# houchenfeng/4DGaussians-fast-train

Hardware: AMD Instinct MI355X
Metric: train-step ms + rasterizer fwd+bwd MGaussians/s @100k pts, 1352×1014 (higher is better)
Workload: dtype f32; 1 GPU; metric: P=100000 Gaussians, 1352x1014, SH deg 3, 1 view/GPU/step, fwd+bwd; global_batch=1, parallelism=views x1 (independent views + RCCL loss all-reduce)

## Files before the change

4dgaussians-fast-train_amd/csrc/capi.hip:

```cpp
#include <stdio.h>
#include <string.h>

#include <algorithm>
#include <string>
#include <vector>

#include "../../include/gs4d.h"
#include "gs4d_internal.h"

namespace gs4d {

static thread_local std::string g_last_error;
static thread_local bool g_profiling = false;
static thread_local int g_stage_repeats = 1;
static thread_local std::vector<std::pair<const char *, hipEvent_t>> g_marks;
static thread_local std::vector<int> g_mark_div;
static thread_local std::vector<std::pair<const char *, float>> g_timings;

static int fail(int code, const std::string &msg) {
    g_last_error = msg;
    return code;
}
int train_fail(int code, const std::string &msg) { return fail(code, msg); }

#define GS4D_HIP(expr)                                                                                                  \
    do {                                                                                                               \
        hipError_t e_ = (expr);                                                                                        \
        if (e_ != hipSuccess)                                                                                          \
            return fail(GS4D_ERR_HIP, std::string(#expr) + ": " + hipGetErrorString(e_));                               \
    } while (0)

#define GS4D_STAGE(name, expr)                                                                                          \
    do {                                                                                                               \
        GS4D_HIP(expr);                                                                                                \
        if (debug) {                                                                                                   \
            hipError_t e_ = hipStreamSynchronize(stream);                                                              \
            if (e_ != hipSuccess)                                                                                      \
                return fail(GS4D_ERR_HIP, std::string("[HIP ERROR] in stage ") + name + ": " + hipGetErrorString(e_)); \
        }                                                                                                              \
        mark(name, stream);                                                                                            \
    } while (0)

#define GS4D_REPEATED_STAGE(name, expr)                                                                                 \
    do {                                                                                                               \
        const int reps_ = g_profiling ? g_stage_repeats : 1;                                                           \
        if (reps_ > 1) mark(name "_pre", stream);                                                                      \
        for (int r_ = 0; r_ < reps_; r_++) GS4D_HIP(expr);                                                             \
        if (debug) {                                                                                                   \
            hipError_t e_ = hipStreamSynchronize(stream);                                                              \
            if (e_ != hipSuccess)                                                                                      \
                return fail(GS4D_ERR_HIP, std::string("[HIP ERROR] in stage ") + name + ": " + hipGetErrorString(e_)); \
        }                                                                                                              \
        mark(name, stream, reps_);                                                                                     \
    } while (0)

static void mark(const char *name, hipStream_t s, int div = 1) {
    if (!g_profiling) return;
    hipEvent_t ev;
    if (hipEventCreate(&ev) != hipSuccess) return;
    (void)hipEventRecord(ev, s);
    g_marks.emplace_back(name, ev);
    g_mark_div.push_back(div);
}
static void begin_marks(hipStream_t s) {
    for (auto &m : g_marks) (void)hipEventDestroy(m.second);
    g_marks.clear();
    g_mark_div.clear();
    mark("begin", s);
}
static void end_marks() {
    if (!g_profiling || g_marks.empty()) return;
    (void)hipEventSynchronize(g_marks.back().second);
    g_timings.clear();
    for (size_t i = 1; i < g_marks.size(); i++) {
        float ms = 0.f;
        (void)hipEventElapsedTime(&ms, g_marks[i - 1].second, g_marks[i].second);
        g_timings.emplace_back(g_marks[i].first, ms / (float)g_mark_div[i]);
    }
    for (auto &m : g_marks) (void)hipEventDestroy(m.second);
    g_marks.clear();
    g_mark_div.clear();
}

static char *carve(char *&p, size_t bytes) {
    char *r = p;
    p += align_up(bytes, 256);
    return r;
}

size_t GeomState::required(int P, int T) { return (size_t)carve(nullptr, P, T).zero + 4 * geom_zero_words(P) + 512; }
GeomState GeomState::carve(char *base, int P, int T) {
    char *p = (char *)align_up((size_t)base, 256);
    const size_t n = (size_t)P;
    GeomState g;
    g.depths = (float *)gs4d::carve(p, 4 * n);
    g.radii = (int *)gs4d::carve(p, 4 * n);
    g.xy = (float2 *)gs4d::carve(p, 8 * n);
    g.conic_opacity = (float4 *)gs4d::carve(p, 16 * n);
    g.splat = (float4 *)gs4d::carve(p, 48 * n);
    g.cov3D = (float *)gs4d::carve(p, 24 * n);
    g.clamped = (uint8_t *)gs4d::carve(p, n);
    g.tiles_touched = (uint32_t *)gs4d::carve(p, 4 * n);
    g.n_inst = (uint32_t *)gs4d::carve(p, 4 * n);
    g.vis_gid = (uint32_t *)gs4d::carve(p, 4 * n);
    g.cand_off = (uint32_t *)gs4d::carve(p, 4 * n + 4);
    g.first_vis = (uint32_t *)gs4d::carve(p, 4 * max_emit_chunks(P, T));
    g.emit_chain = (uint32_t *)gs4d::carve(p, 4 * (max_emit_chunks(P, T) + 64));
    g.zero = (uint32_t *)gs4d::carve(p, 4 * geom_zero_words(P));
    return g;
}

size_t ImageState::required(int W, int H) { return (size_t)carve(nullptr, W, H).order + 4 * (size_t)((W + 15) / 16) * ((H + 15) / 16) + 512; }
ImageState ImageState::carve(char *base, int W, int H) {
    char *p = (char *)align_up((size_t)base, 256);
    const size_t N = (size_t)W * H;
    const size_t T = (size_t)((W + kBlockX - 1) / kBlockX) * ((H + kBlockY - 1) / kBlockY);
    ImageState s;
    s.final_T = (float *)gs4d::carve(p, 4 * N);
    s.n_contrib = (uint32_t *)gs4d::carve(p, 4 * N);
    s.ranges = (uint2 *)gs4d::carve(p, 8 * T);
    s.order = (uint32_t *)gs4d::carve(p, 4 * T);
    return s;
}

static uint32_t higher_msb(uint32_t n) {
    uint32_t msb = sizeof(n) * 4;
    uint32_t step = msb;
    while (step > 1) {
        step /= 2;
        if (n >> msb) msb += step; else msb -= step;
    }
    if (n >> msb) msb++;
    return msb;
}

size_t BinningState::required(int L, int T) {
    BinningState b = carve(nullptr, L, T);
    return (size_t)b.scratch + 4 * binning_zero_words(L, T) + 512;
}
BinningState BinningState::carve(char *base, int L, int T) {
    char *p = (char *)align_up((size_t)base, 256);
    BinningState b;
    b.key_bits = (int)higher_msb((uint32_t)T);
    for (int i = 0; i < 2; i++) {
        b.keys[i] = (uint32_t *)gs4d::carve(p, 4 * (size_t)L);
        b.vals[i] = (uint32_t *)gs4d::carve(p, 4 * (size_t)L);
    }
    b.gid_by_e = (uint32_t *)gs4d::carve(p, 4 * (size_t)L);
    const int final_buf = ((b.key_bits + 7) / 8) & 1;
    b.upos = b.vals[final_buf];
    b.sorted_keys = b.keys[final_buf];
    b.tmp_hi = b.keys[final_buf ^ 1];
    b.tmp_lo = b.vals[final_buf ^ 1];
    b.count_items = gs4d::count_items(L, T);
    b.tile_hist = b.count_items ? (uint32_t *)gs4d::carve(p, 4 * tile_hist_words(L, T)) : nullptr;
    b.scratch = (uint32_t *)gs4d::carve(p, 4 * binning_zero_words(L, T));
    return b;
}

static Args make_args(int P, int D, int M, int W, int H, const float *bg, float scale_modifier, const float *view,
                      const float *proj, const float *campos, float tan_fovx, float tan_fovy, int prefiltered) {
    Args a;
    memset(&a, 0, sizeof(a));
    a.P = P; a.D = D; a.M = M; a.W = W; a.H = H;
    a.gx = (W + kBlockX - 1) / kBlockX;
    a.gy = (H + kBlockY - 1) / kBlockY;
    a.scale_modifier = scale_modifier;
    a.tan_fovx = tan_fovx;
    a.tan_fovy = tan_fovy;
    a.focal_y = H / (2.0f * tan_fovy);
    a.focal_x = W / (2.0f * tan_fovx);
    a.viewmatrix = view;
    a.projmatrix = proj;
    a.campos = campos;
    a.bg = bg;
    a.prefiltered = prefiltered;
    return a;
}

}

using namespace gs4d;

extern "C" {

const char *gs4d_last_error(void) { return g_last_error.c_str(); }
const char *gs4d_version(void) { return "gs4d 0.1.0 gfx950"; }
void gs4d_set_profiling(int enabled) {
    g_profiling = enabled != 0;
    g_stage_repeats = enabled >= 2 ? enabled : 1;
// ... 31 lines not shown
                         uint8_t *present, void *stream_, int view_transposed) {
    hipStream_t stream = (hipStream_t)stream_;
    if (P < 0 || (P > 0 && (!means3D || !viewmatrix || !present))) return fail(GS4D_ERR_ARG, "mark_visible: bad args");
    if (P == 0) return GS4D_OK;
    GS4D_HIP(launch_mark_visible(P, means3D, viewmatrix, view_transposed ? 1 : 0, present, stream));
    return GS4D_OK;
}
int gs4d_mark_visible(int P, const float *means3D, const float *viewmatrix, const float *projmatrix,
                      uint8_t *present, void *stream) {
    return gs4d_mark_visible_ex(P, means3D, viewmatrix, projmatrix, present, stream, 0);
}

int gs4d_debug_effective_opacity(int P, const char *geometry_buffer, float *out, void *stream_) {
    if (P < 0 || (P > 0 && (!geometry_buffer || !out))) return fail(GS4D_ERR_ARG, "debug_effective_opacity: bad args");
    if (P == 0) return GS4D_OK;
    GeomState g = GeomState::carve(const_cast<char *>(geometry_buffer), P, 1);
    GS4D_HIP(launch_effective_opacity(P, g, out, (hipStream_t)stream_));
    return GS4D_OK;
}

int gs4d_debug_tile_lists(int P, int width, int height, int num_rendered, const char *geometry_buffer,
                          const char *binning_buffer, const char *image_buffer, uint32_t *ranges, uint32_t *order,
                          uint32_t *n_emitted, uint32_t *gid, uint32_t *reach, uint32_t *slot, float *depth,
                          void *stream_) {
    hipStream_t stream = (hipStream_t)stream_;
    const int R = num_rendered;
    if (P <= 0 || width <= 0 || height <= 0 || R < 0 || !geometry_buffer || !image_buffer || !ranges || !order ||
        !n_emitted || (R > 0 && (!binning_buffer || !gid || !reach || !slot || !depth)))
        return fail(GS4D_ERR_ARG, "debug_tile_lists: bad args");
    const int T = ((width + kBlockX - 1) / kBlockX) * ((height + kBlockY - 1) / kBlockY);
    GeomState g = GeomState::carve(const_cast<char *>(geometry_buffer), P, T);
    ImageState img = ImageState::carve(const_cast<char *>(image_buffer), width, height);
    GS4D_HIP(hipMemcpyAsync(ranges, img.ranges, sizeof(uint2) * (size_t)T, hipMemcpyDeviceToDevice, stream));
    GS4D_HIP(hipMemcpyAsync(order, img.order, 4 * (size_t)T, hipMemcpyDeviceToDevice, stream));
    if (R == 0) {
        GS4D_HIP(hipMemsetAsync(n_emitted, 0, 4, stream));
        return GS4D_OK;
    }
    BinningState b = BinningState::carve(const_cast<char *>(binning_buffer), R, T);
    GS4D_HIP(hipMemcpyAsync(n_emitted, b.scratch, 4, hipMemcpyDeviceToDevice, stream));
    GS4D_HIP(launch_tile_lists(P, R, g, b, gid, reach, slot, depth, stream));
    return GS4D_OK;
}

int gs4d_forward_aa(gs4d_alloc_fn geometry_alloc, void *geometry_ctx, gs4d_alloc_fn binning_alloc, void *binning_ctx,
                    gs4d_alloc_fn image_alloc, void *image_ctx, int P, int D, int M, const float *background,
                    int width, int height, const float *means3D, const float *shs, const float *colors_precomp,
                    const float *opacities, const float *scales, float scale_modifier, const float *rotations,
                    const float *cov3D_precomp, const float *viewmatrix, const float *projmatrix,
                    const float *cam_pos, float tan_fovx, float tan_fovy, int prefiltered, float *out_color,
                    float *out_depth, int *radii, int debug, void *stream_, int *num_rendered, int view_transposed,
                    int antialiasing) {
    hipStream_t stream = (hipStream_t)stream_;
    *num_rendered = 0;
    if (P < 0 || width <= 0 || height <= 0) return fail(GS4D_ERR_ARG, "forward: P must be >= 0 and the image non-empty");
    if (P == 0) return GS4D_OK;
    if (P >= (1 << 30)) return fail(GS4D_ERR_ARG, "forward: at most 2^30 Gaussians");
    if (!means3D || !opacities || !viewmatrix || !projmatrix || !background || !out_color || !out_depth)
        return fail(GS4D_ERR_ARG, "forward: missing required input");
    if (!colors_precomp && (!shs || !cam_pos))
        return fail(GS4D_ERR_ARG, "forward: provide either SHs (+campos) or precomputed colors");
    if (!colors_precomp && (D < 0 || D > 3 || (D + 1) * (D + 1) > M))
        return fail(GS4D_ERR_ARG, "forward: SH degree must be in [0,3] with (D+1)^2 <= M coefficients");
    if (!cov3D_precomp && (!scales || !rotations))
        return fail(GS4D_ERR_ARG, "forward: provide either scales+rotations or precomputed 3D covariances");
    if (((size_t)rotations & 15) != 0 && rotations) return fail(GS4D_ERR_ARG, "forward: rotations must be 16-byte aligned");

    Args a = make_args(P, D, M, width, height, background, scale_modifier, viewmatrix, projmatrix, cam_pos, tan_fovx,
                       tan_fovy, prefiltered);
    a.view_transposed = view_transposed ? 1 : 0;
    begin_marks(stream);

    if ((int64_t)a.gx * a.gy >= (int64_t)1 << 30) return fail(GS4D_ERR_ARG, "forward: at most 2^30 - 1 tiles");
    const int T = a.gx * a.gy;
    a.exact_div = T >= (1 << 20);
    char *gbuf = geometry_alloc(geometry_ctx, GeomState::required(P, T) + 16);
    if (!gbuf) return fail(GS4D_ERR_ALLOC, "forward: geometry buffer allocation failed");
    GeomState g = GeomState::carve(gbuf, P, T);
    char *ibuf = image_alloc(image_ctx, ImageState::required(width, height));
    if (!ibuf) return fail(GS4D_ERR_ALLOC, "forward: image buffer allocation failed");
    ImageState img = ImageState::carve(ibuf, width, height);
    int *radii_ptr = radii ? radii : g.radii;

    GS4D_HIP(hipMemsetAsync(g.zero, 0, 4 * geom_zero_words(P), stream));
    GS4D_STAGE("preprocess", launch_preprocess(a, means3D, scales, rotations, opacities, shs, cov3D_precomp,
                                               colors_precomp, radii_ptr, g, (int *)(g.zero + kZeroFlag),
                                               antialiasing != 0, stream));

    struct Readback {
        uint32_t *pinned = nullptr;
        hipEvent_t copied = nullptr;
    };
    static thread_local Readback readback[kMaxDevices];
    int dev = 0;
    GS4D_HIP(hipGetDevice(&dev));
    if (dev < 0 || dev >= kMaxDevices) return fail(GS4D_ERR_ARG, "forward: device index out of range");
    Readback &rb = readback[dev];
    if (!rb.pinned) GS4D_HIP(hipHostMalloc((void **)&rb.pinned, 128, hipHostMallocDefault));
    if (!rb.copied) GS4D_HIP(hipEventCreateWithFlags(&rb.copied, hipEventDisableTiming));
    uint32_t *pinned = rb.pinned;
    hipEvent_t copied = rb.copied;
    GS4D_HIP(hipMemcpyAsync(pinned, g.zero, 4 * (kZeroL + 16), hipMemcpyDeviceToHost, stream));
    GS4D_HIP(hipEventRecord(copied, stream));
    GS4D_STAGE("visible_scan", launch_visible_scan(a, g, stream));
    GS4D_HIP(hipEventSynchronize(copied));
    if (prefiltered && pinned[kZeroFlag] != 0)
        return fail(GS4D_ERR_PREFILTERED, "Point is filtered although prefiltered is set. This shouldn't happen!");
    uint64_t L64 = 0;
    for (int i = 0; i < kHistShards; i++) L64 += reinterpret_cast<const uint64_t *>(pinned + kZeroL)[i];
    if (L64 >= (1u << 30)) return fail(GS4D_ERR_ARG, "forward: more than 2^30 tile instances");
    const int L = (int)L64;
    *num_rendered = L;

    char *bbuf = binning_alloc(binning_ctx, BinningState::required(L, T));
    if (!bbuf) return fail(GS4D_ERR_ALLOC, "forward: binning buffer allocation failed");
    BinningState b = BinningState::carve(bbuf, L, T);
    GS4D_STAGE("binning", launch_binning(a, g, radii_ptr, b, L, img, stream));
    GS4D_REPEATED_STAGE("render", launch_render_forward(a, g, b, img, out_color, out_depth, stream));
    end_marks();
    return GS4D_OK;
}

int gs4d_forward_ex(gs4d_alloc_fn geometry_alloc, void *geometry_ctx, gs4d_alloc_fn binning_alloc, void *binning_ctx,
                    gs4d_alloc_fn image_alloc, void *image_ctx, int P, int D, int M, const float *background,
                    int width, int height, const float *means3D, const float *shs, const float *colors_precomp,
                    const float *opacities, const float *scales, float scale_modifier, const float *rotations,
                    const float *cov3D_precomp, const float *viewmatrix, const float *projmatrix,
                    const float *cam_pos, float tan_fovx, float tan_fovy, int prefiltered, float *out_color,
                    float *out_depth, int *radii, int debug, void *stream, int *num_rendered, int view_transposed) {
    return gs4d_forward_aa(geometry_alloc, geometry_ctx, binning_alloc, binning_ctx, image_alloc, image_ctx, P, D, M,
                           background, width, height, means3D, shs, colors_precomp, opacities, scales, scale_modifier,
                           rotations, cov3D_precomp, viewmatrix, projmatrix, cam_pos, tan_fovx, tan_fovy, prefiltered,
                           out_color, out_depth, radii, debug, stream, num_rendered, view_transposed, 0);
}

}

namespace {
struct BackwardCall {
    int P, D, M, R;
    const float *background;
    int width, height;
    const float *means3D, *shs, *colors_precomp, *scales;
    float scale_modifier;
    const float *rotations, *cov3D_precomp, *viewmatrix, *projmatrix, *campos;
    float tan_fovx, tan_fovy;
    const int *radii;
    char *geom_buffer, *binning_buffer, *image_buffer;
    const float *dL_dpix, *dL_ddepth, *dL_dalpha;
    float *dL_dmean2D, *dL_dconic, *dL_dopacity, *dL_dcolor, *dL_dmean3D, *dL_dcov3D, *dL_dsh, *dL_dscale, *dL_drot;
    float *abs_dmean2D;
    gs4d_alloc_fn scratch_alloc;
    void *scratch_ctx;
    int debug;
    void *stream;
    int view_transposed;
    bool need_depth, need_abs;
    const float *aa_opacities = nullptr;
    float *dL_dcamera = nullptr;
};
}

static int backward_impl(const BackwardCall &c) {
    hipStream_t stream = (hipStream_t)c.stream;
    const int debug = c.debug, P = c.P, R = c.R;
    if (P < 0 || R < 0) return fail(GS4D_ERR_ARG, "backward: bad sizes");
    if (c.need_abs && !c.abs_dmean2D) return fail(GS4D_ERR_ARG, "backward_absgrad: missing abs_dmean2D");
    if (P == 0) {
        if (c.dL_dcamera) GS4D_HIP(hipMemsetAsync(c.dL_dcamera, 0, 35 * sizeof(float), stream));
        return GS4D_OK;
    }
    if (c.need_depth && (!c.dL_ddepth || !c.dL_dpix))
        return fail(GS4D_ERR_ARG, "backward_depth: missing dL_ddepth or dL_dpix");
    if (!c.geom_buffer || !c.image_buffer || (R > 0 && !c.binning_buffer) || !c.dL_dpix || !c.means3D)
        return fail(GS4D_ERR_ARG, "backward: missing buffers");
    if (c.shs && (c.D < 0 || c.D > 3 || (c.D + 1) * (c.D + 1) > c.M))
        return fail(GS4D_ERR_ARG, "backward: SH degree must be in [0,3] with (D+1)^2 <= M coefficients");
    if (c.rotations && ((size_t)c.rotations & 15) != 0)
        return fail(GS4D_ERR_ARG, "backward: rotations must be 16-byte aligned");
    if (((size_t)c.dL_drot & 15) != 0) return fail(GS4D_ERR_ARG, "backward: dL_drot must be 16-byte aligned");
    if (!c.viewmatrix || !c.projmatrix || !c.background || (c.shs && !c.campos))
        return fail(GS4D_ERR_ARG, "backward: missing camera inputs");
    const bool depth = c.dL_ddepth != nullptr;
    Args a = make_args(P, c.D, c.M, c.width, c.height, c.background, c.scale_modifier, c.viewmatrix, c.projmatrix,
                       c.campos, c.tan_fovx, c.tan_fovy, 0);
    a.view_transposed = c.view_transposed ? 1 : 0;
    begin_marks(stream);
    const int T = a.gx * a.gy;
    GeomState g = GeomState::carve(c.geom_buffer, P, T);
    ImageState img = ImageState::carve(c.image_buffer, c.width, c.height);
    const int *radii_ptr = c.radii ? c.radii : g.radii;
    const size_t rec_bytes = align_up((size_t)R * kContribStride * sizeof(float), 256);
// ... 324 lines not shown
```

4dgaussians-fast-train_amd/csrc/gs4d_internal.h:

```cpp
#pragma once
#include <hip/hip_runtime.h>
#include <stddef.h>
#include <stdint.h>

#include <type_traits>

#include "gs4d_math.h"

namespace gs4d {

constexpr int kTilePixels = kBlockX * kBlockY;
constexpr float kLog2e = 1.4426950408889634f;
constexpr int kPreprocessBlock = 256;
constexpr int kMaxDevices = 64;
constexpr int kContribStride = 12;

struct GeomState {
    float *depths;
    int *radii;
    float2 *xy;
    float4 *conic_opacity;
    float4 *splat;
    float *cov3D;
    uint8_t *clamped;
    uint32_t *tiles_touched;
    uint32_t *n_inst;
    uint32_t *vis_gid;
    uint32_t *cand_off;
    uint32_t *first_vis;
    uint32_t *emit_chain;
    uint32_t *zero;
    static size_t required(int P, int T);
    static GeomState carve(char *base, int P, int T);
};
constexpr int kZeroFlag = 0, kZeroL = 8, kZeroV = 24, kZeroHist = 64;
constexpr int kHistShards = 8, kMaxPasses = 4;
constexpr int kHistWords = kHistShards * kMaxPasses * 256;

struct ImageState {
    float *final_T;
    uint32_t *n_contrib;
    uint2 *ranges;
    uint32_t *order;
    static size_t required(int W, int H);
    static ImageState carve(char *base, int W, int H);
};

constexpr int kEmitChunk = 2048;
size_t max_emit_chunks(int P, int T);

struct BinningState {
    uint32_t *keys[2];
    uint32_t *vals[2];
    uint32_t *gid_by_e;
    uint32_t *upos;
    uint32_t *sorted_keys;
    uint32_t *tmp_hi, *tmp_lo;
    uint32_t *tile_hist;
    uint32_t *scratch;
    int key_bits;
    int count_items;
    static size_t required(int L, int T);
    static BinningState carve(char *base, int L, int T);
};

struct Args {
    int P, D, M, W, H, gx, gy;
    float scale_modifier, tan_fovx, tan_fovy, focal_x, focal_y;
    const float *viewmatrix, *projmatrix, *campos, *bg;
    int prefiltered;
    int view_transposed;
    int exact_div;
};
__device__ __forceinline__ Mat4 load_mat4(const float *__restrict__ p, bool transposed = false) {
    Mat4 m;
#pragma unroll
    for (int i = 0; i < 16; i++) m.m[i] = transposed ? p[(i & 3) * 4 + (i >> 2)] : p[i];
    return m;
}
__device__ __forceinline__ V3 load_v3(const float *__restrict__ p) { return v3(p[0], p[1], p[2]); }

size_t geom_zero_words(int P);
size_t binning_zero_words(int L, int T);
int count_items(int L, int T);
size_t tile_hist_words(int L, int T);

__device__ __forceinline__ float edge_q(float a, float b2, float c, float X, float y) {
    return __builtin_fmaf(X, __builtin_fmaf(b2, y, a * X), c * y * y);
}
__device__ __forceinline__ float clampf(float v, float lo, float hi) { return fminf(fmaxf(v, lo), hi); }
__device__ __forceinline__ uint32_t half_reach(float mx, float my, float4 co, int tx, int ty, int W, int H) {
    const float a = co.x, b = co.y, c = co.z, o = co.w;
    const int px0 = tx * kBlockX, px1 = min(px0 + kBlockX - 1, W - 1);
    const int y00 = ty * kBlockY, y01 = min(y00 + 7, H - 1), y10 = y00 + 8, y11 = min(y00 + 15, H - 1);
    const uint32_t exists = 1u | (y10 <= y11 ? 2u : 0u);
    if (!(a > 0.f && c > 0.f && a * c - b * b > 0.f)) return exists;
    const float thr = (2.f * 0.693147181f) * __log2f(o * (255.f * 1.001f));
    const float b2 = 2.f * b, ia = __builtin_amdgcn_rcpf(a), ic = __builtin_amdgcn_rcpf(c);
    const float X0 = mx - (float)px1, X1 = mx - (float)px0;
    const float ys0 = -b * X0 * ic, ys1 = -b * X1 * ic;
    const bool xin = X0 <= 0.f && X1 >= 0.f;
    uint32_t r = 0;
#pragma unroll
    for (int h = 0; h < 2; h++) {
        const float Y0 = my - (float)(h ? y11 : y01), Y1 = my - (float)(h ? y10 : y00);
        const float q0 = edge_q(a, b2, c, X0, clampf(ys0, Y0, Y1));
        const float q1 = edge_q(a, b2, c, X1, clampf(ys1, Y0, Y1));
        const float q2 = edge_q(c, b2, a, Y0, clampf(-b * Y0 * ia, X0, X1));
        const float q3 = edge_q(c, b2, a, Y1, clampf(-b * Y1 * ia, X0, X1));
        const float qmin = (xin && Y0 <= 0.f && Y1 >= 0.f) ? 0.f : fminf(fminf(q0, q1), fminf(q2, q3));
        if (qmin <= thr) r |= 1u << h;
    }
    return r & exists;
// ... 93 lines not shown
```

4dgaussians-fast-train_amd/csrc/preprocess.hip:

```cpp
#include "gs4d_internal.h"

namespace gs4d {

template <bool AA>
__global__ __launch_bounds__(kPreprocessBlock) void preprocess_kernel(
    Args a, const float *__restrict__ means3D, const float *__restrict__ scales, const float *__restrict__ rotations,
    const float *__restrict__ opacities, const float *__restrict__ shs, const float *__restrict__ cov3D_precomp,
    const float *__restrict__ colors_precomp, int *__restrict__ radii, GeomState g, int *__restrict__ err_flag) {
    __shared__ uint32_t s_wave[kPreprocessBlock / 64];
    const int idx = blockIdx.x * kPreprocessBlock + threadIdx.x;
    const Mat4 view = load_mat4(a.viewmatrix, a.view_transposed), proj = load_mat4(a.projmatrix);
    uint32_t touched = 0;
    if (idx < a.P) {
        int my_r = 0;
        V3 p_orig = v3(means3D[3 * idx], means3D[3 * idx + 1], means3D[3 * idx + 2]);
        V3 p_view = transformPoint4x3(p_orig, view);
        bool ok = !(p_view.z <= 0.2f);
        if (!ok && a.prefiltered) atomicOr(err_flag, 1);
        float cov3[6];
        float3 cov;
        float det = 0.f;
        if (ok) {
            float4 p_hom = transformPoint4x4(p_orig, proj);
            float p_w = 1.0f / (p_hom.w + 0.0000001f);
            float p_proj_x = p_hom.x * p_w, p_proj_y = p_hom.y * p_w;
            if (cov3D_precomp != nullptr) {
#pragma unroll
                for (int i = 0; i < 6; i++) cov3[i] = cov3D_precomp[6 * (size_t)idx + i];
            } else {
                V3 sc = v3(scales[3 * idx], scales[3 * idx + 1], scales[3 * idx + 2]);
                float4 rot = reinterpret_cast<const float4 *>(rotations)[idx];
                computeCov3D(sc, a.scale_modifier, rot, cov3);
#pragma unroll
                for (int i = 0; i < 6; i++) g.cov3D[6 * (size_t)idx + i] = cov3[i];
            }
            float3 raw;
            cov = computeCov2D(p_orig, a.focal_x, a.focal_y, a.tan_fovx, a.tan_fovy, cov3, view, AA ? &raw : nullptr);
            det = (cov.x * cov.z - cov.y * cov.y);
            ok = det != 0.0f;
            if (ok) {
                float det_inv = 1.f / det;
                float3 conic = make_float3(cov.z * det_inv, -cov.y * det_inv, cov.x * det_inv);
                float mid = 0.5f * (cov.x + cov.z);
                float lambda1 = mid + sqrtf(fmaxf(0.1f, mid * mid - det));
                float lambda2 = mid - sqrtf(fmaxf(0.1f, mid * mid - det));
                float my_radius = ceilf(3.f * sqrtf(fmaxf(lambda1, lambda2)));
                float2 point_image = make_float2(ndc2Pix(p_proj_x, a.W), ndc2Pix(p_proj_y, a.H));
                int x0, y0, x1, y1;
                getRect(point_image.x, point_image.y, (int)my_radius, a.gx, a.gy, x0, y0, x1, y1);
                uint32_t area = (uint32_t)((y1 - y0) * (x1 - x0));
                if (area != 0) {
                    float3 rgb;
                    uint8_t cl = 0;
                    if (colors_precomp == nullptr) {
                        const float *sh = shs + (size_t)idx * a.M * 3;
                        V3 dir = p_orig - load_v3(a.campos);
                        float len = sqrtf(dot(dir, dir));
                        dir = v3(dir.x / len, dir.y / len, dir.z / len);
                        V3 res;
                        if (a.M == 16 && ((size_t)shs & 15) == 0) {
                            float shl[48];
                            const float4 *s4 = reinterpret_cast<const float4 *>(sh);
#pragma unroll
                            for (int q = 0; q < 12; q++) {
                                const float4 v = s4[q];
                                shl[4 * q] = v.x, shl[4 * q + 1] = v.y, shl[4 * q + 2] = v.z, shl[4 * q + 3] = v.w;
                            }
                            res = sh_eval(a.D, shl, dir);
                        } else {
                            res = sh_eval(a.D, sh, dir);
                        }
                        cl = (uint8_t)((res.x < 0) | ((res.y < 0) << 1) | ((res.z < 0) << 2));
                        rgb = make_float3(fmaxf(res.x, 0.0f), fmaxf(res.y, 0.0f), fmaxf(res.z, 0.0f));
                    } else {
                        rgb = make_float3(colors_precomp[3 * idx], colors_precomp[3 * idx + 1],
                                          colors_precomp[3 * idx + 2]);
                    }
                    float opac = opacities[idx];
                    if (AA) opac = opac * aa_factor(raw.x, raw.y, raw.z).s;
                    const float4 co = make_float4(conic.x, conic.y, conic.z, opac);
                    g.clamped[idx] = cl;
                    g.depths[idx] = p_view.z;
                    g.xy[idx] = point_image;
                    g.conic_opacity[idx] = co;
                    float4 *rec = g.splat + 3 * (size_t)idx;
                    const float ga = (-0.5f * co.x) * kLog2e, gb = (-co.y) * kLog2e, gc = (-0.5f * co.z) * kLog2e;
                    const bool pd = ga < 0.f && 4.f * ga * gc - gb * gb > 0.f;
                    rec[0] = make_float4(point_image.x, point_image.y, ga, gb);
                    rec[1] = make_float4(gc, pd ? 1.f : co.w, co.w > 0.f ? 1.0f / co.w : 0.f, p_view.z);
                    rec[2] = make_float4(rgb.x, rgb.y, rgb.z, pd ? log2f(co.w) : 0.f);
                    my_r = (int)my_radius;
                    touched = area;
                }
            }
        }
        radii[idx] = my_r;
        g.tiles_touched[idx] = touched;
        g.n_inst[idx] = 0;
    }
    uint32_t v = touched;
#pragma unroll
    for (int off = 32; off > 0; off >>= 1) v += __shfl_xor(v, off);
    if ((threadIdx.x & 63) == 0) s_wave[threadIdx.x >> 6] = v;
    __syncthreads();
    const int shard = blockIdx.x % kHistShards;
    if (threadIdx.x == 0) {
        uint32_t t = 0;
#pragma unroll
        for (int w = 0; w < kPreprocessBlock / 64; w++) t += s_wave[w];
        if (t) atomicAdd(reinterpret_cast<unsigned long long *>(g.zero + kZeroL) + shard, (unsigned long long)t);
    }
}

hipError_t launch_preprocess(const Args &a, const float *means3D, const float *scales, const float *rotations,
                             const float *opacities, const float *shs, const float *cov3D_precomp,
                             const float *colors_precomp, int *radii, GeomState g, int *err_flag, bool antialiasing,
                             hipStream_t s) {
    const int nblk = (a.P + kPreprocessBlock - 1) / kPreprocessBlock;
    hipLaunchKernelGGL(antialiasing ? preprocess_kernel<true> : preprocess_kernel<false>, dim3(nblk),
                       dim3(kPreprocessBlock), 0, s, a, means3D, scales, rotations, opacities, shs, cov3D_precomp,
                       colors_precomp, radii, g, err_flag);
    return hipGetLastError();
}

__global__ void effective_opacity_kernel(int P, const float4 *__restrict__ conic_opacity, float *__restrict__ out) {
    const int idx = blockIdx.x * blockDim.x + threadIdx.x;
    if (idx < P) out[idx] = conic_opacity[idx].w;
}
hipError_t launch_effective_opacity(int P, GeomState g, float *out, hipStream_t s) {
    hipLaunchKernelGGL(effective_opacity_kernel, dim3((P + 255) / 256), dim3(256), 0, s, P, g.conic_opacity, out);
    return hipGetLastError();
}

__global__ void mark_visible_kernel(int P, const float *__restrict__ means3D, const float *__restrict__ viewmatrix,
                                    int view_transposed,
                                    uint8_t *__restrict__ present) {
    const int idx = blockIdx.x * blockDim.x + threadIdx.x;
    if (idx >= P) return;
    const Mat4 view = load_mat4(viewmatrix, view_transposed);
    V3 p = v3(means3D[3 * idx], means3D[3 * idx + 1], means3D[3 * idx + 2]);
    V3 pv = transformPoint4x3(p, view);
    present[idx] = !(pv.z <= 0.2f);
}

hipError_t launch_mark_visible(int P, const float *means3D, const float *viewmatrix, int view_transposed,
                               uint8_t *present, hipStream_t s) {
    hipLaunchKernelGGL(mark_visible_kernel, dim3((P + 255) / 256), dim3(256), 0, s, P, means3D, viewmatrix,
                       view_transposed, present);
    return hipGetLastError();
}

}
```

4dgaussians-fast-train_amd/csrc/preprocess_backward.hip:

```cpp
#include <algorithm>

#include "gs4d_internal.h"

namespace gs4d {

struct GradOut {
    float *mean2D;
    float4 *conic;
    float *opacity;
    float *color;
    const float4 *conic_opacity;
    float hw, hh;
    float *abs_mean2D;
};
constexpr float kLn2 = 0.6931471805599453f;
template <int NV, bool ABS>
constexpr int n_acc() { return NV + (ABS ? 2 : 0); }
template <int NV, bool ABS>
__device__ __forceinline__ void write_grads(const GradOut &o, uint32_t g, const float *R) {
    const float4 co = o.conic_opacity[g];
    const float op = co.w;
    o.mean2D[3 * g + 0] = o.hw * op * (-co.x * R[1] - co.y * R[2]);
    o.mean2D[3 * g + 1] = o.hh * op * (-co.z * R[2] - co.y * R[1]);
    o.mean2D[3 * g + 2] = 0.f;
// ... 199 lines not shown
#pragma unroll
    for (int i = 0; i < 6; i++) dL_dcov3D[6 * (size_t)idx + i] = dcov[i];
    dL_dscale[3 * idx + 0] = dscale.x;
    dL_dscale[3 * idx + 1] = dscale.y;
    dL_dscale[3 * idx + 2] = dscale.z;
    reinterpret_cast<float4 *>(dL_drot)[idx] = drot;
    if (NV == 10) reinterpret_cast<float *>(const_cast<float4 *>(dL_dconic) + idx)[2] = 0.f;
    return dmean;
}

__device__ __forceinline__ const float *raw_opacities() { return nullptr; }
__device__ __forceinline__ const float *raw_opacities(const float *p) { return p; }
__device__ __forceinline__ const float *raw_opacities(CamRows) { return nullptr; }
__device__ __forceinline__ const float *raw_opacities(const float *p, CamRows) { return p; }
__device__ __forceinline__ float *cam_rows() { return nullptr; }
__device__ __forceinline__ float *cam_rows(const float *) { return nullptr; }
__device__ __forceinline__ float *cam_rows(CamRows c) { return c.rows; }
__device__ __forceinline__ float *cam_rows(const float *, CamRows c) { return c.rows; }
template <class... Raw>
constexpr bool kPackAA = (std::is_same<Raw, const float *>::value || ...);
template <class... Raw>
constexpr bool kPackCam = (std::is_same<Raw, CamRows>::value || ...);

template <int CTRL, int RM>
__device__ __forceinline__ void cam_sum_step(float (&v)[kCamValues]) {
#pragma unroll
    for (int q = 0; q < kCamValues; q++)
        v[q] += __int_as_float(__builtin_amdgcn_update_dpp(0, __float_as_int(v[q]), CTRL, RM, 0xF, false));
}
template <int WAVES>
__device__ __forceinline__ void cam_block_sum(float (&v)[kCamValues], float *__restrict__ row) {
    __shared__ float sums[WAVES * kCamValues];
    cam_sum_step<0x111, 0xF>(v);
    cam_sum_step<0x112, 0xF>(v);
    cam_sum_step<0x114, 0xF>(v);
    cam_sum_step<0x118, 0xF>(v);
    cam_sum_step<0x142, 0xA>(v);
    cam_sum_step<0x143, 0xC>(v);
    if ((threadIdx.x & 63) == 63) {
#pragma unroll
        for (int q = 0; q < kCamValues; q++) sums[(threadIdx.x >> 6) * kCamValues + q] = v[q];
    }
    __syncthreads();
    if (threadIdx.x < kCamValues) {
        float s = sums[threadIdx.x];
#pragma unroll
        for (int w = 1; w < WAVES; w++) s += sums[w * kCamValues + threadIdx.x];
        row[threadIdx.x] = s;
    }
}

template <int NV, bool ABS, class... Raw>
__global__ __launch_bounds__(256) void gaussian_backward_kernel(
    Args a, GeomState g, const int *__restrict__ radii, const float *__restrict__ means3D,
    const float *__restrict__ scales, const float *__restrict__ rotations, const float *__restrict__ cov3Ds,
    const float *dL_dmean2D, const float4 *dL_dconic, float *__restrict__ dL_dmean3D,
    float *__restrict__ dL_dcov3D, float *__restrict__ dL_dscale, float *__restrict__ dL_drot,
    const uint32_t *__restrict__ e_first, const float4 *__restrict__ part, GradOut o,
    Raw... raw) {
    const int idx = blockIdx.x * blockDim.x + threadIdx.x;
    if constexpr (kPackCam<Raw...>) {
        float cam[kCamValues] = {};
        if (idx < a.P) {
            const V3 dmean = gaussian_grads<NV, ABS, kPackAA<Raw...>, true>(
                idx, a, g, radii, means3D, scales, rotations, cov3Ds, dL_dmean2D, dL_dconic, dL_dcov3D, dL_dscale,
                dL_drot, e_first, part, o, raw_opacities(raw...), cam);
            dL_dmean3D[3 * idx + 0] = dmean.x;
            dL_dmean3D[3 * idx + 1] = dmean.y;
            dL_dmean3D[3 * idx + 2] = dmean.z;
        }
        cam_block_sum<4>(cam, cam_rows(raw...) + (size_t)blockIdx.x * kCamRow);
    } else {
        if (idx >= a.P) return;
        const V3 dmean = gaussian_grads<NV, ABS, kPackAA<Raw...>>(idx, a, g, radii, means3D, scales, rotations, cov3Ds, dL_dmean2D, dL_dconic,
                                        dL_dcov3D, dL_dscale, dL_drot, e_first, part, o, raw_opacities(raw...));
        dL_dmean3D[3 * idx + 0] = dmean.x;
        dL_dmean3D[3 * idx + 1] = dmean.y;
        dL_dmean3D[3 * idx + 2] = dmean.z;
    }
}

constexpr int kShThreads = 128, kShRow = 49;

template <bool kVec4, int NV, bool ABS, class... Raw>
__global__ __launch_bounds__(kShThreads) void gaussian_sh_backward_kernel(
    Args a, GeomState g, const int *__restrict__ radii, const float *__restrict__ means3D,
    const float *__restrict__ scales, const float *__restrict__ rotations, const float *__restrict__ cov3Ds,
    const float *dL_dmean2D, const float4 *dL_dconic, float *__restrict__ dL_dmean3D,
    float *__restrict__ dL_dcov3D, float *__restrict__ dL_dscale, float *__restrict__ dL_drot,
    const uint32_t *__restrict__ e_first, const float4 *__restrict__ part, GradOut o, const float *__restrict__ shs,
    const uint8_t *__restrict__ clamped, const float *dL_dcolor, float *__restrict__ dL_dsh,
    Raw... raw) {
    __shared__ float tile[kShThreads * kShRow];
    const int g0 = blockIdx.x * kShThreads;
    const int n = min(kShThreads, a.P - g0), row = 3 * a.M, rowl = min(row, 48);
    const size_t base = (size_t)g0 * row;
    const int total = n * row;
    if (kVec4) {
        const float4 *s4 = reinterpret_cast<const float4 *>(shs + base);
        for (int i = threadIdx.x; i < total / 4; i += kShThreads) {
            const int r = i / 12, c = (i - r * 12) * 4;
            const float4 v = s4[i];
            float *t = tile + r * kShRow + c;
            t[0] = v.x, t[1] = v.y, t[2] = v.z, t[3] = v.w;
        }
    } else {
        for (int i = threadIdx.x; i < total; i += kShThreads) {
            const int r = i / row, c = i - r * row;
            if (c < 48) tile[r * kShRow + c] = shs[base + i];
        }
    }
    V3 dmean = v3(0, 0, 0);
    const int idx = g0 + threadIdx.x;
    constexpr bool CAM = kPackCam<Raw...>;
    float cam[CAM ? kCamValues : 1] = {};
    if ((int)threadIdx.x < n)
        dmean = gaussian_grads<NV, ABS, kPackAA<Raw...>, CAM>(idx, a, g, radii, means3D, scales, rotations, cov3Ds, dL_dmean2D,
                                                              dL_dconic, dL_dcov3D, dL_dscale, dL_drot, e_first, part, o,
                                                              raw_opacities(raw...), cam);
    __syncthreads();
    if ((int)threadIdx.x < n) {
        float *trow = tile + threadIdx.x * kShRow;
        float shl[48];
#pragma unroll
        for (int k = 0; k < 48; k++) {
            shl[k] = k < rowl ? trow[k] : 0.f;
            if (k < rowl) trow[k] = 0.f;
        }
        if (radii[idx] > 0) {
            const uint8_t cl = clamped[idx];
            const V3 dRGB = v3(dL_dcolor[3 * idx] * ((cl & 1) ? 0.f : 1.f),
                               dL_dcolor[3 * idx + 1] * ((cl & 2) ? 0.f : 1.f),
                               dL_dcolor[3 * idx + 2] * ((cl & 4) ? 0.f : 1.f));
            const V3 m = v3(means3D[3 * idx], means3D[3 * idx + 1], means3D[3 * idx + 2]);
            const V3 dm = sh_backward(a.D, shl, m - load_v3(a.campos), dRGB, trow);
            dmean = dmean + dm;
            if constexpr (CAM) {
                cam[24] = -dm.x;
                cam[25] = -dm.y;
                cam[26] = -dm.z;
            }
        }
        dL_dmean3D[3 * idx + 0] = dmean.x;
        dL_dmean3D[3 * idx + 1] = dmean.y;
        dL_dmean3D[3 * idx + 2] = dmean.z;
    }
    if constexpr (CAM) cam_block_sum<kShThreads / 64>(cam, cam_rows(raw...) + (size_t)blockIdx.x * kCamRow);
    __syncthreads();
    if (kVec4) {
        float4 *d4 = reinterpret_cast<float4 *>(dL_dsh + base);
        for (int i = threadIdx.x; i < total / 4; i += kShThreads) {
            const int r = i / 12, c = (i - r * 12) * 4;
            const float *t = tile + r * kShRow + c;
            d4[i] = make_float4(t[0], t[1], t[2], t[3]);
        }
    } else {
        for (int i = threadIdx.x; i < total; i += kShThreads) {
            const int r = i / row, c = i - r * row;
            dL_dsh[base + i] = c < 48 ? tile[r * kShRow + c] : 0.f;
        }
    }
}

static size_t cam_rows_max(int P) { return ((size_t)P + kShThreads - 1) / kShThreads; }
size_t contrib_scratch_bytes(int R, int P, bool camera) {
    const size_t nw = ((size_t)R + 63) / 64;
    return align_up(nw * 2 * 3 * sizeof(float4), 256) + align_up(4 * (size_t)P, 256) + 256 +
           (camera ? align_up(cam_rows_max(P) * kCamRow * sizeof(float), 256) : 0);
}

static GradOut grad_out(const Args &a, GeomState g, float *dL_dmean2D, float4 *dL_dconic, float *dL_dopacity,
                        float *dL_dcolor, float *abs_dmean2D) {
    return GradOut{dL_dmean2D, dL_dconic, dL_dopacity, dL_dcolor, g.conic_opacity, 0.5f * a.W, 0.5f * a.H, abs_dmean2D};
}
static float4 *scratch_part(char *scratch) { return (float4 *)scratch; }
static uint32_t *scratch_e_first(char *scratch, int R) {
    const size_t nw = ((size_t)R + 63) / 64;
    return (uint32_t *)(scratch + align_up(nw * 2 * 3 * sizeof(float4), 256));
}
static float *scratch_cam_rows(char *scratch, int R, int P) {
    return (float *)((char *)scratch_e_first(scratch, R) + align_up(4 * (size_t)P, 256));
}

template <int NV, bool ABS>
static hipError_t contrib_reduce(const Args &a, GeomState g, BinningState b, int R, const float *contrib,
                                 char *scratch, float *dL_dmean2D, float4 *dL_dconic, float *dL_dopacity,
                                 float *dL_dcolor, float *abs_dmean2D, hipStream_t s) {
    if (R == 0) return hipSuccess;
// ... 66 lines not shown
```

Baseline: 274.7 MGaussians/s.

## Replace preprocess atomics and memset with per-block slots; batch SH tile loads

Preprocess now writes each block's tile-instance count and a prefilter-fail flag into a per-block 64-bit slot instead of doing sharded global atomics. It also zeroes the zero-region inside the kernel, so the separate memset launch is dropped. The host copies back all slots and sums them, which adds a larger readback and a host-side loop in exchange for one fewer launch and no atomics. Separately, the SH backward kernel issues all twelve float4 loads into registers before storing them to shared memory, to increase memory-level parallelism at the cost of register pressure.

Result: no change. 276.0 MGaussians/s, median of 6 (+0.5%).

```diff
diff --git a/4dgaussians-fast-train_amd/csrc/capi.hip b/4dgaussians-fast-train_amd/csrc/capi.hip
--- a/4dgaussians-fast-train_amd/csrc/capi.hip
+++ b/4dgaussians-fast-train_amd/csrc/capi.hip
@@ -106,6 +106,7 @@
     g.cand_off = (uint32_t *)gs4d::carve(p, 4 * n + 4);
     g.first_vis = (uint32_t *)gs4d::carve(p, 4 * max_emit_chunks(P, T));
     g.emit_chain = (uint32_t *)gs4d::carve(p, 4 * (max_emit_chunks(P, T) + 64));
+    g.slots = (uint64_t *)gs4d::carve(p, 8 * (size_t)std::min(preprocess_blocks(P), kSlotMaxBlocks));
     g.zero = (uint32_t *)gs4d::carve(p, 4 * geom_zero_words(P));
     return g;
 }
@@ -303,13 +304,16 @@
     ImageState img = ImageState::carve(ibuf, width, height);
     int *radii_ptr = radii ? radii : g.radii;
 
-    GS4D_HIP(hipMemsetAsync(g.zero, 0, 4 * geom_zero_words(P), stream));
+    const bool slots = preprocess_slots(P);
+    const int nblk = preprocess_blocks(P);
+    if (!slots) GS4D_HIP(hipMemsetAsync(g.zero, 0, 4 * geom_zero_words(P), stream));
     GS4D_STAGE("preprocess", launch_preprocess(a, means3D, scales, rotations, opacities, shs, cov3D_precomp,
                                                colors_precomp, radii_ptr, g, (int *)(g.zero + kZeroFlag),
                                                antialiasing != 0, stream));
 
     struct Readback {
         uint32_t *pinned = nullptr;
+        size_t bytes = 0;
         hipEvent_t copied = nullptr;
     };
     static thread_local Readback readback[kMaxDevices];
@@ -317,18 +321,36 @@
     GS4D_HIP(hipGetDevice(&dev));
     if (dev < 0 || dev >= kMaxDevices) return fail(GS4D_ERR_ARG, "forward: device index out of range");
     Readback &rb = readback[dev];
-    if (!rb.pinned) GS4D_HIP(hipHostMalloc((void **)&rb.pinned, 128, hipHostMallocDefault));
+    const size_t copy_bytes = slots ? 8 * (size_t)nblk : 4 * (size_t)(kZeroL + 16);
+    if (rb.bytes < copy_bytes) {
+        if (rb.pinned) GS4D_HIP(hipHostFree(rb.pinned));
+        rb.pinned = nullptr, rb.bytes = 0;
+        const size_t want = align_up(std::max<size_t>(copy_bytes, 4096), 4096);
+        GS4D_HIP(hipHostMalloc((void **)&rb.pinned, want, hipHostMallocDefault));
+        rb.bytes = want;
+    }
     if (!rb.copied) GS4D_HIP(hipEventCreateWithFlags(&rb.copied, hipEventDisableTiming));
     uint32_t *pinned = rb.pinned;
     hipEvent_t copied = rb.copied;
-    GS4D_HIP(hipMemcpyAsync(pinned, g.zero, 4 * (kZeroL + 16), hipMemcpyDeviceToHost, stream));
+    GS4D_HIP(hipMemcpyAsync(pinned, slots ? (const void *)g.slots : (const void *)g.zero, copy_bytes,
+                            hipMemcpyDeviceToHost, stream));
     GS4D_HIP(hipEventRecord(copied, stream));
     GS4D_STAGE("visible_scan", launch_visible_scan(a, g, stream));
     GS4D_HIP(hipEventSynchronize(copied));
-    if (prefiltered && pinned[kZeroFlag] != 0)
+    uint64_t L64 = 0;
+    bool filtered = false;
+    if (slots) {
+        const uint64_t *slot = reinterpret_cast<const uint64_t *>(pinned);
+        for (int i = 0; i < nblk; i++) {
+            L64 += slot[i] & ~kSlotFlag;
+            filtered |= (slot[i] & kSlotFlag) != 0;
+        }
+    } else {
+        filtered = pinned[kZeroFlag] != 0;
+        for (int i = 0; i < kHistShards; i++) L64 += reinterpret_cast<const uint64_t *>(pinned + kZeroL)[i];
+    }
+    if (prefiltered && filtered)
         return fail(GS4D_ERR_PREFILTERED, "Point is filtered although prefiltered is set. This shouldn't happen!");
-    uint64_t L64 = 0;
-    for (int i = 0; i < kHistShards; i++) L64 += reinterpret_cast<const uint64_t *>(pinned + kZeroL)[i];
     if (L64 >= (1u << 30)) return fail(GS4D_ERR_ARG, "forward: more than 2^30 tile instances");
     const int L = (int)L64;
     *num_rendered = L;
diff --git a/4dgaussians-fast-train_amd/csrc/gs4d_internal.h b/4dgaussians-fast-train_amd/csrc/gs4d_internal.h
--- a/4dgaussians-fast-train_amd/csrc/gs4d_internal.h
+++ b/4dgaussians-fast-train_amd/csrc/gs4d_internal.h
@@ -12,6 +12,10 @@
 constexpr int kTilePixels = kBlockX * kBlockY;
 constexpr float kLog2e = 1.4426950408889634f;
 constexpr int kPreprocessBlock = 256;
+constexpr int kSlotMaxBlocks = 4096;
+inline int preprocess_blocks(int P) { return (P + kPreprocessBlock - 1) / kPreprocessBlock; }
+inline bool preprocess_slots(int P) { return preprocess_blocks(P) <= kSlotMaxBlocks; }
+constexpr uint64_t kSlotFlag = 1ull << 63;
 constexpr int kMaxDevices = 64;
 constexpr int kContribStride = 12;
 
@@ -29,6 +33,7 @@
     uint32_t *cand_off;
     uint32_t *first_vis;
     uint32_t *emit_chain;
+    uint64_t *slots;
     uint32_t *zero;
     static size_t required(int P, int T);
     static GeomState carve(char *base, int P, int T);
diff --git a/4dgaussians-fast-train_amd/csrc/preprocess.hip b/4dgaussians-fast-train_amd/csrc/preprocess.hip
--- a/4dgaussians-fast-train_amd/csrc/preprocess.hip
+++ b/4dgaussians-fast-train_amd/csrc/preprocess.hip
@@ -2,13 +2,19 @@
 
 namespace gs4d {
 
-template <bool AA>
+template <bool AA, bool SLOTS>
 __global__ __launch_bounds__(kPreprocessBlock) void preprocess_kernel(
     Args a, const float *__restrict__ means3D, const float *__restrict__ scales, const float *__restrict__ rotations,
     const float *__restrict__ opacities, const float *__restrict__ shs, const float *__restrict__ cov3D_precomp,
-    const float *__restrict__ colors_precomp, int *__restrict__ radii, GeomState g, int *__restrict__ err_flag) {
+    const float *__restrict__ colors_precomp, int *__restrict__ radii, GeomState g, int *__restrict__ err_flag,
+    int nzero) {
     __shared__ uint32_t s_wave[kPreprocessBlock / 64];
+    __shared__ uint32_t s_bad[kPreprocessBlock / 64];
     const int idx = blockIdx.x * kPreprocessBlock + threadIdx.x;
+    if constexpr (SLOTS) {
+        for (int i = idx; i < nzero; i += gridDim.x * kPreprocessBlock) g.zero[i] = 0u;
+    }
+    bool bad = false;
     const Mat4 view = load_mat4(a.viewmatrix, a.view_transposed), proj = load_mat4(a.projmatrix);
     uint32_t touched = 0;
     if (idx < a.P) {
@@ -16,7 +22,10 @@
         V3 p_orig = v3(means3D[3 * idx], means3D[3 * idx + 1], means3D[3 * idx + 2]);
         V3 p_view = transformPoint4x3(p_orig, view);
         bool ok = !(p_view.z <= 0.2f);
-        if (!ok && a.prefiltered) atomicOr(err_flag, 1);
+        if (!ok && a.prefiltered) {
+            if (SLOTS) bad = true;
+            else atomicOr(err_flag, 1);
+        }
         float cov3[6];
         float3 cov;
         float det = 0.f;
@@ -101,14 +110,22 @@
     uint32_t v = touched;
 #pragma unroll
     for (int off = 32; off > 0; off >>= 1) v += __shfl_xor(v, off);
-    if ((threadIdx.x & 63) == 0) s_wave[threadIdx.x >> 6] = v;
+    const bool wave_bad = SLOTS && __ballot(bad) != 0ull;
+    if ((threadIdx.x & 63) == 0) {
+        s_wave[threadIdx.x >> 6] = v;
+        if (SLOTS) s_bad[threadIdx.x >> 6] = wave_bad;
+    }
     __syncthreads();
-    const int shard = blockIdx.x % kHistShards;
     if (threadIdx.x == 0) {
-        uint32_t t = 0;
+        uint32_t t = 0, f = 0;
 #pragma unroll
-        for (int w = 0; w < kPreprocessBlock / 64; w++) t += s_wave[w];
-        if (t) atomicAdd(reinterpret_cast<unsigned long long *>(g.zero + kZeroL) + shard, (unsigned long long)t);
+        for (int w = 0; w < kPreprocessBlock / 64; w++) {
+            t += s_wave[w];
+            if (SLOTS) f |= s_bad[w];
+        }
+        if (SLOTS) g.slots[blockIdx.x] = (uint64_t)t | (f ? kSlotFlag : 0ull);
+        else if (t) atomicAdd(reinterpret_cast<unsigned long long *>(g.zero + kZeroL) + blockIdx.x % kHistShards,
+                              (unsigned long long)t);
     }
 }
 
@@ -116,10 +133,12 @@
                              const float *opacities, const float *shs, const float *cov3D_precomp,
                              const float *colors_precomp, int *radii, GeomState g, int *err_flag, bool antialiasing,
                              hipStream_t s) {
-    const int nblk = (a.P + kPreprocessBlock - 1) / kPreprocessBlock;
-    hipLaunchKernelGGL(antialiasing ? preprocess_kernel<true> : preprocess_kernel<false>, dim3(nblk),
-                       dim3(kPreprocessBlock), 0, s, a, means3D, scales, rotations, opacities, shs, cov3D_precomp,
-                       colors_precomp, radii, g, err_flag);
+    const auto kernel = preprocess_slots(a.P)
+                            ? (antialiasing ? preprocess_kernel<true, true> : preprocess_kernel<false, true>)
+                            : (antialiasing ? preprocess_kernel<true, false> : preprocess_kernel<false, false>);
+    hipLaunchKernelGGL(kernel, dim3(preprocess_blocks(a.P)), dim3(kPreprocessBlock), 0, s, a, means3D, scales,
+                       rotations, opacities, shs, cov3D_precomp, colors_precomp, radii, g, err_flag,
+                       (int)geom_zero_words(a.P));
     return hipGetLastError();
 }
 
diff --git a/4dgaussians-fast-train_amd/csrc/preprocess_backward.hip b/4dgaussians-fast-train_amd/csrc/preprocess_backward.hip
--- a/4dgaussians-fast-train_amd/csrc/preprocess_backward.hip
+++ b/4dgaussians-fast-train_amd/csrc/preprocess_backward.hip
@@ -305,6 +305,27 @@
 
 constexpr int kShThreads = 128, kShRow = 49;
 
+template <int THREADS>
+__device__ __forceinline__ void sh_span_load(float4 (&v)[12], const float4 *__restrict__ s4, int total4) {
+#pragma unroll
+    for (int k = 0; k < 12; k++) {
+        const int i = (int)threadIdx.x + k * THREADS;
+        v[k] = i < total4 ? s4[i] : make_float4(0.f, 0.f, 0.f, 0.f);
+    }
+}
+template <int THREADS>
+__device__ __forceinline__ void sh_span_store(float *__restrict__ tile, const float4 (&v)[12], int total4) {
+#pragma unroll
+    for (int k = 0; k < 12; k++) {
+        const int i = (int)threadIdx.x + k * THREADS;
+        if (i < total4) {
+            const int r = i / 12, c = (i - r * 12) * 4;
+            float *t = tile + r * kShRow + c;
+            t[0] = v[k].x, t[1] = v[k].y, t[2] = v[k].z, t[3] = v[k].w;
+        }
+    }
+}
+
 template <bool kVec4, int NV, bool ABS, class... Raw>
 __global__ __launch_bounds__(kShThreads) void gaussian_sh_backward_kernel(
     Args a, GeomState g, const int *__restrict__ radii, const float *__restrict__ means3D,
@@ -320,13 +341,9 @@
     const size_t base = (size_t)g0 * row;
     const int total = n * row;
     if (kVec4) {
-        const float4 *s4 = reinterpret_cast<const float4 *>(shs + base);
-        for (int i = threadIdx.x; i < total / 4; i += kShThreads) {
-            const int r = i / 12, c = (i - r * 12) * 4;
-            const float4 v = s4[i];
-            float *t = tile + r * kShRow + c;
-            t[0] = v.x, t[1] = v.y, t[2] = v.z, t[3] = v.w;
-        }
+        float4 span[12];
+        sh_span_load<kShThreads>(span, reinterpret_cast<const float4 *>(shs + base), total / 4);
+        sh_span_store<kShThreads>(tile, span, total / 4);
     } else {
         for (int i = threadIdx.x; i < total; i += kShThreads) {
             const int r = i / row, c = i - r * row;
```
